# highlando/optconpy

Measured on AMD Instinct MI355X. Metric: ADI shift-solves/sec (wall-clock to feedback K in ms_per_step), higher is better.
Workload: dtype f64

## Files before the change

### include/ricadi.h

```cpp
#ifndef RICADI_H
#define RICADI_H

#include <stdint.h>

#ifdef __cplusplus
extern "C" {
#endif

#define RICADI_OK 0
#define RICADI_EINVAL (-1)
#define RICADI_EHIP (-2)
#define RICADI_ENOCONV (-3)
#define RICADI_EBREAKDOWN (-4)
#define RICADI_ESTATE (-5)

typedef struct ricadi_ctx ricadi_ctx;

#define RICADI_MAX_HIERARCHY_LEVELS 6

typedef struct ricadi_opts {
  double gmres_tol;
  int gmres_restart;
  int gmres_maxit;
  int bj_block;
// ... 39 lines not shown
                        const int32_t* a_rowptr, const int32_t* a_col, const double* a_val,
                        const int32_t* e_rowptr, const int32_t* e_col, const double* e_val,
                        const int32_t* j_rowptr, const int32_t* j_col, const double* j_val);

int ricadi_clear_cache(ricadi_ctx* ctx);

int ricadi_set_dims(ricadi_ctx* ctx, int nv);

int ricadi_set_lowrank(ricadi_ctx* ctx, const double* U, const double* V, int q);

int ricadi_spmm(ricadi_ctx* ctx, double alpha, double beta,
                const double* X, int m, double* Y);

int ricadi_precond_apply(ricadi_ctx* ctx, double alpha, double beta,
                         const double* R, int m, double* Z);

#define RICADI_PCF_H16 (1 << 0)
#define RICADI_PCF_X32 (1 << 1)
#define RICADI_PCF_MID32 (1 << 2)
#define RICADI_PCF_B16 (1 << 3)
#define RICADI_PCF_RESTRICT_SHIFT 4
#define RICADI_PCF_COARSE_SHIFT 6
#define RICADI_PCF_PFUSED (1 << 8)
#define RICADI_PCF_PSPLIT (1 << 9)
#define RICADI_PCF_FIRST_SHIFT 10
#define RICADI_PCF_LAST_SHIFT 12
#define RICADI_PCF_FOLDED (1 << 14)
#define RICADI_PCF_VANKA (1 << 15)
#define RICADI_PCF_TWO_KS_SHIFT 16
#define RICADI_PCF_RECT_KS_SHIFT 24
int ricadi_precond_apply_batch_dev(ricadi_ctx* ctx, int ng, const double* alphas, const double* betas,
                                   const double* dR, int64_t r_stride, int m, const int32_t* active,
                                   int nactive, double* dZ, int* form_out);

#define RICADI_OA_X32 1
#define RICADI_OA_Y32 2
#define RICADI_OA_LOWRANK 4
#define RICADI_OA_RESIDUAL 8
int ricadi_op_apply_batch_dev(ricadi_ctx* ctx, int ng, const double* alphas, const double* betas, const double* dX,
                              int64_t x_stride, int m, const int32_t* active, int nactive, int flags, double alpha,
                              const double* dR, int64_t r_stride, double beta_r, double* dY, int64_t y_stride,
                              int* variant_out);

int ricadi_precond_structure(ricadi_ctx* ctx, int level, int32_t* sizes_out, int32_t* bv_ptr, int32_t* bv_rows,
                             int32_t* bp_ptr, int32_t* bp_rows, int32_t* aggof, int32_t* p_rp, int32_t* p_ci,
                             double* p_v);

int ricadi_precond_vanka(ricadi_ctx* ctx, int level, int32_t* sizes_out, int32_t* colour_ptr, int32_t* patch_idx);

int ricadi_shift_solve(ricadi_ctx* ctx, double alpha, double beta,
                       const double* R, const double* Rp, int m,
                       double* X_out, int* iters_out, double* relres_out);

int ricadi_lyap_adi(ricadi_ctx* ctx, const double* shifts, int nshifts,
                    const double* W, int m, const ricadi_adi_params* prm,
                    double* Z_out, int* c_out, double* stats_out);

int ricadi_ric_newtonadi(ricadi_ctx* ctx, const double* shifts, int nshifts,
                         const double* B, int nb, const double* W, int mw,
                         const double* Z0, int c0, const double* oldB,
                         const ricadi_adi_params* prm,
                         double* Z_out, int zcap, int* c_out, double* stats_out);

int ricadi_compress(ricadi_ctx* ctx, const double* Z, int c, double thresh, int kmax,
                    double* Zc_out, int* k_out, double* sv_out);

// ... 59 lines not shown
#define RICADI_TK_ITER_SPLIT 18
#define RICADI_TK_PC_VANKA 19
int ricadi_time_kernel_dev(ricadi_ctx* ctx, int which, int ng, const double* alphas,
                           const double* betas, int m, int nvec, int reps,
                           double* ms_per_launch);

int ricadi_qr(ricadi_ctx* ctx, const double* Z, int c, double* Q_out, double* R_out);

int ricadi_project_pencil(ricadi_ctx* ctx, const double* Q, int k, double* HA, double* HE);
int ricadi_project_pencil_dev(ricadi_ctx* ctx, const double* dQ, int k, double* dHA, double* dHE);

int ricadi_setup_info(ricadi_ctx* ctx, int* out, int nout);

int ricadi_dense_inverse_batch(ricadi_ctx* ctx, int k, int nb, double* A, int* route_out);

int ricadi_time_qr_dev(ricadi_ctx* ctx, const double* dZ, int c, int reps, double* ms_per_call);

int ricadi_time_gram_dev(ricadi_ctx* ctx, const double* dZ, int c, double* dG, int reps,
                         double* ms_per_launch);

int ricadi_set_recycle(ricadi_ctx* ctx, int depth);

typedef int (*ricadi_allgather_fn)(void* user, const void* send_dev, void* recv_dev,
                                   int64_t bytes_per_rank);
int ricadi_set_exchange(ricadi_ctx* ctx, int rank, int world, ricadi_allgather_fn fn, void* user,
                        void* send_dev, void* recv_dev, int64_t send_capacity);

int ricadi_rccl_unique_id(void* id_out, int bytes);
int ricadi_set_exchange_rccl(ricadi_ctx* ctx, int rank, int world, const void* unique_id, void* comm,
                             int64_t send_capacity);
int ricadi_exchange_count(ricadi_ctx* ctx, int64_t* count_out);

int ricadi_host_deal(const double* shifts, int nshifts, int world, int32_t* owner_out);
int ricadi_host_sa_criterion(int nv, const int32_t* a_rowptr, const int32_t* a_col, const double* a_val,
                             double* rowsum_ratio_out, double* skew_ratio_out, int* on_out);
int ricadi_host_plan_levels(int nv, int np, const int32_t* a_rowptr, const int32_t* a_col, const double* a_val,
                            const int32_t* e_rowptr, const int32_t* e_col, const double* e_val,
                            const int32_t* j_rowptr, const int32_t* j_col, const double* j_val,
                            const ricadi_opts* opts, int32_t* out);
int ricadi_host_plan_hierarchy(int nv, int np, const int32_t* a_rowptr, const int32_t* a_col, const double* a_val,
                               const int32_t* e_rowptr, const int32_t* e_col, const double* e_val,
                               const int32_t* j_rowptr, const int32_t* j_col, const double* j_val,
                               const ricadi_opts* opts, int32_t* nlevels_out, int32_t* levels_out,
                               int32_t* smoothed_out);
int ricadi_host_saddle_tiles(int nv, int np, const int32_t* a_rowptr, const int32_t* a_col, const double* a_val,
                             const int32_t* e_rowptr, const int32_t* e_col, const double* e_val,
                             const int32_t* j_rowptr, const int32_t* j_col, const double* j_val,
                             const ricadi_opts* opts, int32_t* sizes_out, int32_t* rows2, int32_t* rp2,
                             int32_t* cols2, uint16_t* lidx, uint16_t* lidx_ms, double* vAJ, double* vE,
                             int32_t* perm, int32_t* s_rp, int32_t* s_ci, double* s_src);
int ricadi_host_vanka_patches(int nv, int np, const int32_t* j_rowptr, const int32_t* j_col, const double* j_val,
                              int32_t* sizes_out, int32_t* colour_ptr, int32_t* patch_idx);
int ricadi_host_aggregate(int n, const int32_t* rowptr, const int32_t* col,
                          int bsize, int32_t* blk_out);
int ricadi_host_cauchy(const double* shifts, int g, double* rinv_out, double* cinv1_out);

#ifdef __cplusplus
}
#endif
#endif
```

### optconpy_amd/_lib.py

```python
from __future__ import annotations

import ctypes as C
import os

import numpy as np
import scipy.sparse as sps

_HERE = os.path.dirname(os.path.abspath(__file__))
LIB_PATH = os.environ.get("RICADI_LIB", os.path.join(_HERE, "libricadi_hip.so"))

RICADI_OK = 0
RICADI_ENOCONV = -3
MAX_M = 128
ABI_VERSION = 403


class RicadiOpts(C.Structure):
    _fields_ = [("gmres_tol", C.c_double), ("gmres_restart", C.c_int),
                ("gmres_maxit", C.c_int), ("bj_block", C.c_int), ("agg_v", C.c_int),
                ("agg_p", C.c_int), ("coarse_max", C.c_int), ("use_coarse", C.c_int),
                ("max_levels", C.c_int), ("verbose", C.c_int), ("compress_qr", C.c_int),
                ("hierarchy", C.c_int), ("child_smoother", C.c_int), ("child_damping", C.c_double)]


class RicadiAdiParams(C.Structure):
    _fields_ = [("adi_max_steps", C.c_int), ("adi_newZ_reltol", C.c_double),
                ("nwtn_max_steps", C.c_int), ("nwtn_upd_reltol", C.c_double),
                ("nwtn_upd_abstol", C.c_double), ("project_w", C.c_int),
                ("verbose", C.c_int), ("compress_cols", C.c_int), ("sweep_width", C.c_int)]


_dp = C.POINTER(C.c_double)
_ip = C.POINTER(C.c_int32)
_vp = C.c_void_p
_up = C.POINTER(C.c_uint16)

SIGNATURES = {
    "ricadi_last_error": (C.c_char_p, []),
    "ricadi_version": (C.c_int, []),
    "ricadi_sizeof_opts": (C.c_int, []),
    "ricadi_sizeof_adi_params": (C.c_int, []),
    "ricadi_struct_signature": (C.c_char_p, []),
    "ricadi_default_opts": (None, [C.POINTER(RicadiOpts)]),
    "ricadi_default_adi_params": (None, [C.POINTER(RicadiAdiParams)]),
    "ricadi_create": (C.c_int, [C.c_int, C.POINTER(_vp)]),
    "ricadi_destroy": (C.c_int, [_vp]),
    "ricadi_set_opts": (C.c_int, [_vp, C.POINTER(RicadiOpts)]),
# ... 27 lines not shown
    "ricadi_spmm_dev": (C.c_int, [_vp, C.c_double, C.c_double, _vp, C.c_int, _vp]),
    "ricadi_shift_solve_dev": (C.c_int, [_vp, C.c_double, C.c_double, _vp, C.c_int, _vp,
                                         C.POINTER(C.c_int), _dp]),
    "ricadi_shift_solve_batch_dev": (C.c_int, [_vp, C.c_int, _dp, _dp, _vp, C.c_int64, C.c_int, _vp,
                                               C.POINTER(C.c_int), _dp]),
    "ricadi_time_spmm_batch_dev": (C.c_int, [_vp, C.c_int, _dp, _dp, _vp, C.c_int, _vp, C.c_int,
                                             C.POINTER(C.c_double)]),
    "ricadi_sweep_recombine_dev": (C.c_int, [_vp, C.c_int, _vp, C.c_int, _dp, _dp, _vp, _vp,
                                             C.POINTER(C.c_double)]),
    "ricadi_sweep_recombine_slots_dev": (C.c_int, [_vp, C.c_int, C.c_int, _vp, C.c_int, _dp, _dp, _vp, _vp,
                                                   C.POINTER(C.c_double), _dp]),
    "ricadi_apply_e_dev": (C.c_int, [_vp, C.c_double, _vp, C.c_int, _vp]),
    "ricadi_lincomb_dev": (C.c_int, [_vp, C.c_int, C.c_int, C.c_int, _vp, C.c_int64, _dp, _vp]),
    "ricadi_gain_dev": (C.c_int, [_vp, C.c_double, _vp, C.c_int, C.c_int, _vp, C.c_int, _vp]),
    "ricadi_panel_norms_dev": (C.c_int, [_vp, _vp, C.c_int, C.c_int, _dp, _dp]),
    "ricadi_time_spmm_dev": (C.c_int, [_vp, C.c_double, C.c_double, _vp, C.c_int, _vp, C.c_int,
                                       _dp]),
    "ricadi_time_kernel_dev": (C.c_int, [_vp, C.c_int, C.c_int, _dp, _dp, C.c_int, C.c_int, C.c_int,
                                         C.POINTER(C.c_double)]),
    "ricadi_qr": (C.c_int, [_vp, _dp, C.c_int, _dp, _dp]),
    "ricadi_project_pencil": (C.c_int, [_vp, _dp, C.c_int, _dp, _dp]),
    "ricadi_project_pencil_dev": (C.c_int, [_vp, _vp, C.c_int, _vp, _vp]),
    "ricadi_setup_info": (C.c_int, [_vp, C.POINTER(C.c_int), C.c_int]),
    "ricadi_time_qr_dev": (C.c_int, [_vp, _vp, C.c_int, C.c_int, C.POINTER(C.c_double)]),
    "ricadi_time_gram_dev": (C.c_int, [_vp, _vp, C.c_int, _vp, C.c_int, _dp]),
    "ricadi_set_recycle": (C.c_int, [_vp, C.c_int]),
    "ricadi_set_exchange": (C.c_int, [_vp, C.c_int, C.c_int, _vp, _vp, _vp, _vp, C.c_int64]),
    "ricadi_rccl_unique_id": (C.c_int, [_vp, C.c_int]),
    "ricadi_set_exchange_rccl": (C.c_int, [_vp, C.c_int, C.c_int, _vp, _vp, C.c_int64]),
    "ricadi_exchange_count": (C.c_int, [_vp, C.POINTER(C.c_int64)]),
    "ricadi_dense_inverse_batch": (C.c_int, [_vp, C.c_int, C.c_int, _dp, C.POINTER(C.c_int)]),
    "ricadi_precond_apply_batch_dev": (C.c_int, [_vp, C.c_int, _dp, _dp, _vp, C.c_int64, C.c_int, _ip, C.c_int,
                                                 _vp, C.POINTER(C.c_int)]),
    "ricadi_precond_structure": (C.c_int, [_vp, C.c_int, _ip, _ip, _ip, _ip, _ip, _ip, _ip, _ip, _dp]),
    "ricadi_op_apply_batch_dev": (C.c_int, [_vp, C.c_int, _dp, _dp, _vp, C.c_int64, C.c_int, _ip, C.c_int, C.c_int,
                                            C.c_double, _vp, C.c_int64, C.c_double, _vp, C.c_int64,
                                            C.POINTER(C.c_int)]),
    "ricadi_host_saddle_tiles": (C.c_int, [C.c_int, C.c_int, _ip, _ip, _dp, _ip, _ip, _dp, _ip, _ip, _dp,
                                           C.POINTER(RicadiOpts), _ip, _ip, _ip, _ip, _up, _up, _dp, _dp, _ip, _ip,
                                           _ip, _dp]),
    "ricadi_host_deal": (C.c_int, [_dp, C.c_int, C.c_int, _ip]),
    "ricadi_host_sa_criterion": (C.c_int, [C.c_int, _ip, _ip, _dp, C.POINTER(C.c_double), C.POINTER(C.c_double),
                                           C.POINTER(C.c_int)]),
    "ricadi_host_plan_levels": (C.c_int, [C.c_int, C.c_int, _ip, _ip, _dp, _ip, _ip, _dp, _ip, _ip, _dp,
                                          C.POINTER(RicadiOpts), _ip]),
    "ricadi_host_plan_hierarchy": (C.c_int, [C.c_int, C.c_int, _ip, _ip, _dp, _ip, _ip, _dp, _ip, _ip, _dp,
                                             C.POINTER(RicadiOpts), _ip, _ip, _ip]),
    "ricadi_host_aggregate": (C.c_int, [C.c_int, _ip, _ip, C.c_int, _ip]),
    "ricadi_host_vanka_patches": (C.c_int, [C.c_int, C.c_int, _ip, _ip, _dp, _ip, _ip, _ip]),
    "ricadi_precond_vanka": (C.c_int, [_vp, C.c_int, _ip, _ip, _ip]),
    "ricadi_host_cauchy": (C.c_int, [_dp, C.c_int, _dp, _dp]),
}

EXCHANGE_FN = C.CFUNCTYPE(C.c_int, _vp, _vp, _vp, C.c_int64)

_lib = None


def load():
    global _lib
    if _lib is not None:
        return _lib
    if not os.path.exists(LIB_PATH):
        raise RuntimeError(
            "libricadi_hip.so is missing ({0}); build it with "
            "`python -c 'import __graft_entry__ as g; g.build()'` -- there is no "
# ... 465 lines not shown

    def shift_solve_batch_dev(self, alphas, betas, r_ptr, r_stride, m, x_ptr, strict=True):
        al = np.ascontiguousarray(alphas, dtype=np.float64)
        be = np.ascontiguousarray(betas, dtype=np.float64)
        ng = al.size
        its = (C.c_int * ng)()
        rr = np.zeros((ng, m))
        rc = self._lib.ricadi_shift_solve_batch_dev(self._h, ng, _d(al), _d(be), r_ptr,
                                                    int(r_stride), m, x_ptr, its, _d(rr))
        _chk(rc, allow_noconv=not strict)
        return list(its), rr

    def time_spmm_batch_dev(self, alphas, betas, x_ptr, m, y_ptr, reps):
        al = np.ascontiguousarray(alphas, dtype=np.float64)
        be = np.ascontiguousarray(betas, dtype=np.float64)
        ms = C.c_double(0.0)
        _chk(self._lib.ricadi_time_spmm_batch_dev(self._h, al.size, _d(al), _d(be), x_ptr, m, y_ptr,
                                                  reps, C.byref(ms)))
        return ms.value

    TK = dict(spmm=0, block_v=1, block_p=2, coarse=3, spmm_sy=4, dots=5, update_dots=6, update=7,
              precond=8, restrict=9, pc_restrict=10, pc_coarse=11, pc_sy_prows=12, pc_two_term=13,
              pc_jprod=14, pc_schur=15, pc_rect=16, iter=17, iter_split=18, pc_vanka=19)

    def time_kernel_dev(self, which, alphas, betas, m, nvec=7, reps=100):
        al = np.ascontiguousarray(alphas, dtype=np.float64)
        be = np.ascontiguousarray(betas, dtype=np.float64)
        ms = C.c_double(0.0)
        _chk(self._lib.ricadi_time_kernel_dev(self._h, int(self.TK.get(which, which)), al.size, _d(al),
                                              _d(be), int(m), int(nvec), int(reps), C.byref(ms)))
        return ms.value

    def setup_info(self):
        a = (C.c_int * 30)()
        _chk(self._lib.ricadi_setup_info(self._h, a, 30))
        return dict(zip(("nv", "np", "nbv", "nbp", "bs", "kc", "spmm_row_blocks", "spmm_max_cols", "levels",
                         "dense_coarse", "fp16_vector_input", "rect_ks", "two_term_ks", "np_", "nnz_j",
                         "nnz_sy", "nnz_restriction", "coarse_route", "k1_variant", "fp32_intermediate", "fp32_operator_output",
                         "child_smoother", "vanka_colours", "vanka_patches", "vanka_largest_patch", "vanka_dropped",
                         "vanka_lone_patches", "hierarchy", "hierarchy_levels", "hierarchy_dense"),
                        list(a)))

    def dense_inverse_batch(self, mats):
        A = np.ascontiguousarray(mats, dtype=np.float64).copy()
        if A.ndim != 3 or A.shape[1] != A.shape[2]:
            raise ValueError("mats must be nb x k x k")
        route = C.c_int(-1)
        _chk(self._lib.ricadi_dense_inverse_batch(self._h, A.shape[1], A.shape[0], _d(A), C.byref(route)))
        return A, int(route.value)

    PCF_RESTRICT = {0: None, 1: "rowwave", 2: "csr16", 3: "csr64"}
    PCF_COARSE = {0: None, 1: "child", 2: "dense"}
    PCF_FIRST = {0: None, 1: "two32", 2: "two_term", 3: "plain"}
    PCF_LAST = {0: None, 1: "rect32", 2: "rect", 3: "csr_in"}

    @classmethod
    def decode_precond_form(cls, w):
        w &= 0xFFFFFFFF
        return dict(h16=bool(w & 1), x32=bool(w & 2), mid32=bool(w & 4), b16=bool(w & 8),
                    restrict=cls.PCF_RESTRICT[(w >> 4) & 3], coarse=cls.PCF_COARSE[(w >> 6) & 3],
                    pfused=bool(w & (1 << 8)), psplit=bool(w & (1 << 9)), first=cls.PCF_FIRST[(w >> 10) & 3],
                    last=cls.PCF_LAST[(w >> 12) & 3], folded=bool(w & (1 << 14)), vanka=bool(w & (1 << 15)),
                    two_term_ks=(w >> 16) & 255,
                    rect_ks=(w >> 24) & 255)

    def precond_apply_batch_dev(self, alphas, betas, r_ptr, r_stride, m, z_ptr, active=None):
        al = np.ascontiguousarray(alphas, dtype=np.float64)
        be = np.ascontiguousarray(betas, dtype=np.float64)
        act = None if active is None else np.ascontiguousarray(active, dtype=np.int32)
        form = C.c_int(-1)
        _chk(self._lib.ricadi_precond_apply_batch_dev(self._h, al.size, _d(al), _d(be), r_ptr, int(r_stride), int(m),
                                                      None if act is None else _i(act),
                                                      0 if act is None else act.size, z_ptr, C.byref(form)))
        return self.decode_precond_form(form.value)

    OA_X32, OA_Y32, OA_LOWRANK, OA_RESIDUAL = 1, 2, 4, 8

    def op_apply_batch_dev(self, alphas, betas, x_ptr, x_stride, m, y_ptr, y_stride, active=None, flags=0,
                           alpha=1.0, r_ptr=None, r_stride=0, beta_r=0.0):
        al = np.ascontiguousarray(alphas, dtype=np.float64)
        be = np.ascontiguousarray(betas, dtype=np.float64)
        act = None if active is None else np.ascontiguousarray(active, dtype=np.int32)
        var = C.c_int(-1)
        _chk(self._lib.ricadi_op_apply_batch_dev(self._h, al.size, _d(al), _d(be), x_ptr, int(x_stride), int(m),
                                                 None if act is None else _i(act), 0 if act is None else act.size,
                                                 int(flags), float(alpha), r_ptr, int(r_stride), float(beta_r),
                                                 y_ptr, int(y_stride), C.byref(var)))
        return int(var.value)

    def precond_structure(self, level=0):
        sz = np.zeros(16, dtype=np.int32)
        nul = [None] * 8
        _chk(self._lib.ricadi_precond_structure(self._h, int(level), _i(sz), *nul))
        nv, np_, nbv, nbp, bs, kc, kcv, kcp, sa, nnzp, child, folded, rect, p32, agg_v, agg_p = (int(x) for x in sz)
        n = nv + np_
        out = dict(bv_ptr=np.zeros(nbv + 1, np.int32), bv_rows=np.zeros(nv, np.int32),
                   bp_ptr=np.zeros(nbp + 1, np.int32), bp_rows=np.zeros(np_, np.int32),
                   aggof=np.zeros(n if kc > 0 else 0, np.int32), p_rp=np.zeros(n + 1, np.int32),
                   p_ci=np.zeros(nnzp, np.int32), p_v=np.zeros(nnzp))
        ptr = lambda a: _d(a) if a.dtype == np.float64 else _i(a)
        _chk(self._lib.ricadi_precond_structure(self._h, int(level), _i(sz), *[ptr(out[k]) for k in (
            "bv_ptr", "bv_rows", "bp_ptr", "bp_rows", "aggof", "p_rp", "p_ci", "p_v")]))
        P = (sps.csr_matrix((out.pop("p_v"), out.pop("p_ci"), out.pop("p_rp")), shape=(n, kc)) if kc > 0 else None)
        if nbp == 0:
            out["bp_ptr"] = np.zeros(1, np.int32)
        out.update(nv=nv, np=np_, nbv=nbv, nbp=nbp, bs=bs, kc=kc, kcv=kcv, kcp=kcp, smoothed=bool(sa), P=P,
                   child=bool(child), folded=bool(folded), rect=bool(rect), precond32=bool(p32), agg_v=agg_v,
# ... 88 lines not shown

def _vanka_records(call):
    sz = np.zeros(8, dtype=np.int32)
    _chk(call(_i(sz), None, None))
    ncol, npat = int(sz[0]), int(sz[1])
    cp = np.zeros(ncol + 1, dtype=np.int32)
    idx = np.full((npat, 64), -1, dtype=np.int32)
    _chk(call(_i(sz), _i(cp), _i(idx)))
    return dict(colours=ncol, patches=npat, pressure_patches=int(sz[2]), largest=int(sz[3]), dropped=int(sz[4]),
                lone=int(sz[5]), lone_patches=int(sz[6]), colour_ptr=cp, patch_idx=idx)


def host_vanka_patches(nv, J):
    J = sps.csr_matrix(J, dtype=np.float64)
    if J.shape[1] != nv:
        raise ValueError("J has the wrong number of columns")
    rp = np.ascontiguousarray(J.indptr, dtype=np.int32)
    ci = np.ascontiguousarray(J.indices, dtype=np.int32)
    v = np.ascontiguousarray(J.data, dtype=np.float64)
    lib = load()
    return _vanka_records(lambda sz, cp, pi: lib.ricadi_host_vanka_patches(int(nv), J.shape[0], _i(rp), _i(ci),
                                                                           _d(v), sz, cp, pi))


def host_aggregate(pattern, bsize):
    rp, ci, _, sh = as_csr(pattern)
    blk = np.empty(sh[0], dtype=np.int32)
    nb = load().ricadi_host_aggregate(sh[0], _i(rp), _i(ci), int(bsize), _i(blk))
    if nb < 0:
        _chk(nb)
    return blk, nb


def host_deal(shifts, world):
    sh = np.ascontiguousarray(shifts, dtype=np.float64)
    owner = np.empty(sh.size, dtype=np.int32)
    _chk(load().ricadi_host_deal(_d(sh), sh.size, int(world), _i(owner)))
    return owner


def host_cauchy(shifts):
    sh = np.ascontiguousarray(shifts, dtype=np.float64)
    g = sh.size
    rinv = np.empty((g, g))
    c1 = np.empty(g)
    _chk(load().ricadi_host_cauchy(_d(sh), g, _d(rinv), _d(c1)))
    return rinv, c1


def host_plan_levels(calA, calE, J, **opts):
    a, e, j = as_csr(calA), as_csr(calE), as_csr(J)
    o = default_opts(**opts)
    out = np.zeros(5, dtype=np.int32)
    _chk(load().ricadi_host_plan_levels(a[3][0], j[3][0], _i(a[0]), _i(a[1]), _d(a[2]), _i(e[0]), _i(e[1]), _d(e[2]),
                                        _i(j[0]), _i(j[1]), _d(j[2]), C.byref(o), _i(out)))
    return dict(levels=int(out[0]), kc=int(out[1]), kcv=int(out[2]), kcp=int(out[3]), smoothed=bool(out[4]))


PLAN_KEYS = ("nv", "np", "kv", "kp", "agg_v", "agg_p", "has_child", "dense_dim")
MAX_HIERARCHY_LEVELS = 6


def host_plan_hierarchy(calA, calE, J, **opts):
    a, e, j = as_csr(calA), as_csr(calE), as_csr(J)
    o = default_opts(**opts)
    nlev = np.zeros(1, dtype=np.int32)
# ... 45 lines not shown
```

### optconpy_amd/csrc/ricadi_ctx.h

```cpp
#pragma once
#include <rccl/rccl.h>
#include <rocsolver/rocsolver.h>

#include <chrono>
#include <cmath>
#include <future>
#include <numeric>
#include <cstdio>
#include <cstdlib>
#include <cstring>
#include <memory>
#include <tuple>

#include "ricadi_internal.h"

namespace ricadi {

extern thread_local std::string g_err;

struct HipError {
  std::string msg;
};
#define HIPCHK(expr)                                                                      \
  do {                                                                                    \
// ... 169 lines not shown
  DArr<double> v;
  void upload(const HostCsr& h, hipStream_t st) {
    nrows = h.nrows;
    rp.upload(h.rp, st);
    ci.upload(h.ci, st);
    v.upload(h.v, st);
  }
};

struct Exec {
  hipStream_t st = nullptr;
  rocblas_handle rb = nullptr;
  DevPool* pool = nullptr;
  int* info = nullptr;
  int* flag = nullptr;
};

struct Switches {
  bool precond64 = false;
  bool basis64 = false;
  bool basis32 = false;
  bool timing = false;
  bool debug_sweeps = false;
  bool smw = true;
  bool wide_split = true;
  double sa_omega = 0.5;
  bool sweep_meta = true;
  bool ms_spmm = true;
  bool ms_force = false;
  bool w32 = true;
  bool x32_always = true;
  bool blocks16 = true;
  bool rowwave = true;
  bool mid32 = true;
  bool coarse_pipe = true;
  bool lowsync = true;
  bool split = true;
  bool setup_overlap = true;
};

}

using namespace ricadi;

struct ricadi_ctx {
  int dev = 0;
  hipStream_t st = nullptr;
  rocblas_handle rb = nullptr;
  std::unique_ptr<ricadi_ctx> child;
  bool borrowed = false;
  int levels = 2;
  ricadi_opts opts;
  Switches sw;
  bool has_op = false;
  int nv = 0, np = 0, n = 0;
  int bs = 32, nbv = 0, nbp = 0, kc = 0;
  int agg_v = 0, agg_p = 0;
  size_t snnz = 0;
  DArr<int> s_rp, s_ci;
  DArr<double> srcA, srcE, srcJ;
  DevCsr A, E, J, JT;
  DArr<int> bv_ptr, bv_rows, bp_ptr, bp_rows, jd_ptr, jd_vblk;
  DArr<int> ps_meta;
  DArr<int> sw_meta;
  int sw_stride = 0, sw_in_rect = 0, sw_in_two = 0;
  DArr<double> bvA, bvE, jd_val;
// ... 1 lines not shown
  bool ady_ok = false;
  int ady_ks = 0;
  DArr<int> cy_ptr, cy_cols;
  DArr<double> cy_dA, cy_dE, cy_dJ, cy_dT;
  bool sa = false;
  DArr<int> pt_rp, pt_ci;
  DArr<double> pt_v;
  bool vanka = false;
  VankaPatches vk;
  DArr<int> vk_idx;
  bool gt_ok = false;
  int gt_ks = 0;
  DArr<int> gt_ptr, gt_cols;
  DArr<double> gt_jtd;
  DArr<double> E0, EM, EJ, ones;
  size_t synnz = 0;
  int sy_chunk = 16;
  DArr<int> sy_rp, sy_ci;
  DArr<double> sy_A, sy_E, sy_J;
  int syb_max_cols = 0;
  bool syb_ok = false;
  DArr<int> syb_rp2, syb_cols2, syb_perm;
  DArr<uint16_t> syb_lidx;
  int sb_nblk = 0, sb_max_cols = 0, sb_max_nnz = 0;
  bool sb_ok = false;
  DArr<int> sb_perm;
  DArr<int> sb_rows2, sb_rp2, sb_cols2, sb_colsm2;
  DArr<uint16_t> sb_lidx;
  DArr<double> sbAJ, sbE, sybAJ, sybE;
  DArr<uint16_t> sb_lidx_ms, syb_lidx_ms;
  bool ms_ok = false;
  int w32_last = -1;
  int mid32_last = -1;
  int q = 0;
  DArr<double> U, V, lrc, scratch;
  long lr_epoch = 0;
  DArr<double> smw_rhs, smw_x, smw_cap;
  DArr<double> split_b, split_x;
  DArr<double> sweep_u, sweep_t, sweep_coef, sweep_part;
  std::map<std::pair<double, double>, std::unique_ptr<ShiftData>> cache;
  int wcols = 0, wrestart = 0;
  DArr<double> basis, vcur, wv, zv, r2, tp, rc, ec, xs, bvec, pw1, pw2;
  DArr<float> basisf, zbasisf;
  DArr<float> wv32;
  bool basis32 = true;
  bool basis16 = true;
  bool precond32 = true;
  DArr<double> partial, h1, h2, H, cs, sn, g, scale, resid, yv, bnorm2, nrm2;
  DArr<double> ls_partial, ls_coef;
  DArr<int> flag, ipiv, info;
  DArr<double*> eptrs;
  DArr<double> gj_cb, gj_rp, gj_rb, gj_d;
  DArr<double*> gj_ptrs;
  double** gj_hptrs = nullptr;
  size_t gj_hcap = 0;
  DArr<int> flag2;
  double* h_resid = nullptr;
  hipEvent_t ev_res[2] = {nullptr, nullptr};
  hipStream_t st_half = nullptr;
  hipEvent_t ev_res_half[2] = {nullptr, nullptr};
  hipEvent_t ev_fork = nullptr, ev_join = nullptr;
  DArr<double> Z;
  int zc = 0, zld = 0;
  DevPool pool;
  hipStream_t st2 = nullptr;
  rocblas_handle rb2 = nullptr;
// ... 56 lines not shown
```

### optconpy_amd/csrc/ricadi_host.cpp

```cpp
#include <array>
#include <cmath>
#include <cstdio>
#include <cstdlib>
#include <cstring>
#include <numeric>
#include <stdexcept>

#include "ricadi_internal.h"

namespace ricadi {

HostCsr make_csr(int nrows, int ncols, const int32_t* rp, const int32_t* ci, const double* v) {
  HostCsr a;
  a.nrows = nrows;
  a.ncols = ncols;
  a.rp.assign(rp, rp + nrows + 1);
  const int nnz = rp[nrows];
  a.ci.assign(ci, ci + nnz);
  a.v.assign(v, v + nnz);
  sort_rows(a);
  return a;
}

void sort_rows(HostCsr& a) {
// ... 1159 lines not shown
    };
    out(rows2, r.sb_rows2, (size_t)nb * 32);
    out(rp2, r.sb_rp2, (size_t)nb * 33);
    out(cols2, r.sb_cols2, (size_t)nb * mc);
    out(lidx, hs.sb_lidx, nnz);
    out(perm, hs.sb_perm, nnz);
    out(s_rp, hs.s_rp, (size_t)hs.n + 1);
    out(s_ci, hs.s_ci, nnz);
    if (s_src) {
      out(s_src, hs.s_srcA, nnz);
      out(s_src + nnz, hs.s_srcE, nnz);
      out(s_src + 2 * nnz, hs.s_srcJ, nnz);
    }
    if (r.ms_ok) {
      out(lidx_ms, r.sb_lidx_ms, nnz);
      out(vAJ, r.sbAJ, nnz);
      out(vE, r.sbE, nnz);
    }
  } catch (...) {
    ricadi::set_error("ricadi_host_saddle_tiles: exception");
    return RICADI_EINVAL;
  }
  return RICADI_OK;
}

int ricadi_host_deal(const double* shifts, int ns, int world, int32_t* owner_out) {
  if (!shifts || !owner_out || ns < 1 || world < 1) {
    ricadi::set_error("ricadi_host_deal: bad argument");
    return RICADI_EINVAL;
  }
  return ricadi::deal_shifts(shifts, ns, world, owner_out);
}

int ricadi_host_cauchy(const double* shifts, int g, double* rinv_out, double* cinv1_out) {
  if (!shifts || !rinv_out || !cinv1_out) {
    ricadi::set_error("ricadi_host_cauchy: bad argument");
    return RICADI_EINVAL;
  }
  int rc = ricadi::cauchy_data(shifts, g, rinv_out, cinv1_out);
  if (rc == RICADI_EBREAKDOWN)
    ricadi::set_error("ricadi_host_cauchy: Cauchy matrix not positive definite "
                      "(shifts must be distinct, negative and few)");
  return rc;
}

}
```

### optconpy_amd/csrc/ricadi_internal.h

```cpp
#pragma once
#include <hip/hip_runtime.h>

#include <algorithm>
#include <cstddef>
#include <cstdint>
#include <map>
#include <string>
#include <utility>
#include <vector>

#include "../../include/ricadi.h"

#define RICADI_MAX_M 128
#define RICADI_MAX_GROUPS 16

namespace ricadi {

struct HostCsr {
  int nrows = 0, ncols = 0;
  std::vector<int> rp, ci;
  std::vector<double> v;
  size_t nnz() const { return ci.size(); }
};
HostCsr make_csr(int nrows, int ncols, const int32_t* rp, const int32_t* ci, const double* v);
// ... 133 lines not shown
  const int* meta = nullptr;
  int stride = 0, in_off = 0;
};

struct LowRankArgs {
  const double* U = nullptr;
  const double* c = nullptr;
  size_t gsc = 0;
  int q = 0, nrows = 0;
};

struct CsrInArgs {
  const int* rp = nullptr;
  const int* ci = nullptr;
  GroupPtrs v = {};
  const double* src = nullptr;
  size_t gss = 0;
  const double* base = nullptr;
  size_t gsb = 0;
  double scale = 1.0;
};

struct Seg2 {
  const int* iptr = nullptr;
  const int* irows = nullptr;
  const int* moff = nullptr;
  int kstride = 0;
  const double* in = nullptr;
  size_t gs = 0;
  const _Float16* in16 = nullptr;
};

bool spmm_rowwave_pays(int nrows, size_t nnz);
void launch_spmm_rowwave(hipStream_t st, const GroupTab& gt, int nrows, const int* rp, const int* ci,
                         const GroupPtrs& vals, const double* x, const _Float16* x16, size_t gsx, double* y, size_t gsy,
                         int m, bool kb = false);
__host__ __device__ inline size_t rckb_index(int j, int c, int k) {
  return j < (k & ~3) ? ((size_t)(j >> 2) * 16 + c) * 4 + (j & 3) : (size_t)j * 16 + c;
}

void launch_spmm_h(hipStream_t st, const GroupTab& gt, int nrows, const int* rp, const int* ci,
                   const GroupPtrs& vals, const double* x, const _Float16* x16, int ldx, size_t gsx, double* y, int ldy,
                   size_t gsy, const _Float16* r16, int ldr, size_t gsr, double alpha, double beta_r, int m, int chunk);
void launch_spmm_b(hipStream_t st, const GroupTab& gt, int nrows, const int* rp, const int* ci,
                   const GroupPtrs& vals, const double* x, int ldx, size_t gsx, const int* xmap,
                   double* y, int ldy, size_t gsy, const double* r, int ldr, size_t gsr,
                   double alpha, double beta_r, int m, const LowRankArgs& lr = LowRankArgs(),
                   int chunk = 16);
void launch_spmm_blocked_b(hipStream_t st, const GroupTab& gt, int nblk, const int* rows2,
                           const int* rp2, const int* cols2, const uint16_t* lidx,
                           const GroupPtrs& vals, const double* x, int ldx, size_t gsx, double* y,
                           int ldy, size_t gsy, const double* r, int ldr, size_t gsr, double alpha,
                           double beta_r, int m, int max_cols,
                           const LowRankArgs& lr = LowRankArgs());
bool spmm_blocked_ms_ok(int m, int max_cols, size_t panel_rows);
void launch_spmm_blocked_x32(hipStream_t st, const GroupTab& gt, int nblk, const int* rows2, const int* rp2,
                             const int* cols2, const uint16_t* lidx, const GroupPtrs& vals, const float* x, int ldx,
                             size_t gsx, double* y, int ldy, size_t gsy, double alpha, int m, int max_cols, float* y32 = nullptr);
void launch_spmm_blocked_ms_x32(hipStream_t st, const GroupTab& gt, const double* alphas, const double* betas,
                                int nblk, const int* rows2, const int* rp2, const int* cols2, const uint16_t* lidx,
                                const double* vAJ, const double* vE, const float* x, int ldx, size_t gsx, double* y,
                                int ldy, size_t gsy, double alpha, int m, int max_cols, float* y32 = nullptr);
void launch_spmm_blocked_ms(hipStream_t st, const GroupTab& gt, const double* alphas, const double* betas,
                            int nblk, const int* rows2, const int* rp2, const int* cols2,
                            const uint16_t* lidx, const double* vAJ, const double* vE,
                            const double* x, int ldx, size_t gsx, double* y, int ldy, size_t gsy,
                            const double* r, int ldr, size_t gsr, double alpha, double beta_r, int m,
                            int max_cols);
void launch_axpby_b(hipStream_t st, const GroupTab& gt, size_t n, double a, const double* x,
// ... 193 lines not shown
```

### optconpy_amd/csrc/ricadi_spmm.hip

```cpp
#include "ricadi_device.h"

namespace ricadi {

__device__ __forceinline__ double lowrank_term(const LowRankArgs& lr, const double* __restrict__ lrc,
                                               int row, int col, int m) {
  const double* __restrict__ u = lr.U + (size_t)row * lr.q;
  double s = 0.0;
  for (int k = 0; k < lr.q; ++k) s = fma(u[k], lrc[k * m + col], s);
  return s;
}

template <int CPL, int CHK, class XT = double, class RT = double>
__global__ __launch_bounds__(256) void spmm_kernel_v2(
    GroupTab gt, int nrows, const int* __restrict__ rp, const int* __restrict__ ci,
    GroupPtrs vals, const XT* __restrict__ x, int ldx, size_t gsx,
    const int* __restrict__ xmap, double* __restrict__ y, int ldy, size_t gsy,
    const RT* __restrict__ r, int ldr, size_t gsr, double alpha, double beta_r,
    const double* __restrict__ rowscale, int m, LowRankArgs lr) {
  const int grp = gt.gid[blockIdx.z];
  const double* __restrict__ val = vals.p[grp];
  x += (size_t)grp * gsx;
  y += (size_t)grp * gsy;
  if (r) r += (size_t)grp * gsr;
  const double* __restrict__ lrc = lr.c + (size_t)grp * lr.gsc;
  const int nwg = gridDim.x, orig = blockIdx.x;
  const int qd = nwg >> 3, rm = nwg & 7, xcd = orig & 7;
  const int blk = (xcd < rm ? xcd * (qd + 1) : rm * (qd + 1) + (xcd - rm) * qd) + (orig >> 3);
  const int g = threadIdx.x & 15;
  const int row = blk * 16 + (threadIdx.x >> 4);
  const bool live = row < nrows;
  double acc[CPL];
  int colx[CPL];
// ... 183 lines not shown
        acc[1] = fma(myv[u], a.y, acc[1]);
        acc[2] = fma(myv[u], b.x, acc[2]);
        acc[3] = fma(myv[u], b.y, acc[3]);
        acc[4] = fma(myv[u], c2.x, acc[4]);
        acc[5] = fma(myv[u], c2.y, acc[5]);
        acc[6] = fma(myv[u], d.x, acc[6]);
        acc[7] = fma(myv[u], d.y, acc[7]);
      }
    }
  }
#pragma unroll
  for (int t = 0; t < 8; ++t) {
    double v = acc[t];
    v += rw_dpp<0xB1>(v);
    v += rw_dpp<0x4E>(v);
    v += rw_dpp<0x141>(v);
    v += rw_dpp<0x140>(v);
    v += __shfl_xor(v, 16, 64);
    acc[t] = v;
  }
  if (KB && row < (nrows & ~3)) {
    double v = acc[0];
#pragma unroll
    for (int t = 1; t < 8; ++t) v = e == t ? acc[t] : v;
    if (e < 8) y[rckb_index(row, h * 8 + e, nrows)] = v;
  } else if (e == 0) {
    double2* o = reinterpret_cast<double2*>(y + (size_t)row * 16 + h * 8);
    o[0] = make_double2(acc[0], acc[1]);
    o[1] = make_double2(acc[2], acc[3]);
    o[2] = make_double2(acc[4], acc[5]);
    o[3] = make_double2(acc[6], acc[7]);
  }
}
bool spmm_rowwave_pays(int nrows, size_t nnz) { return nrows > 0 && nnz >= (size_t)32 * nrows; }
void launch_spmm_rowwave(hipStream_t st, const GroupTab& gt, int nrows, const int* rp, const int* ci,
                         const GroupPtrs& vals, const double* x, const _Float16* x16, size_t gsx, double* y, size_t gsy,
                         int m, bool kb) {
  if (nrows <= 0 || m != 16 || gt.ng <= 0) return;
  dim3 grid((nrows + 3) / 4, 1, gt.ng), block(256);
#define RW_LAUNCH(XT, KB, X) \
  hipLaunchKernelGGL((spmm_rowwave_kernel<XT, KB>), grid, block, 0, st, gt, nrows, rp, ci, vals, X, gsx, y, gsy)
  if (x16 && kb) RW_LAUNCH(_Float16, true, x16);
  else if (x16) RW_LAUNCH(_Float16, false, x16);
  else if (kb) RW_LAUNCH(double, true, x);
  else RW_LAUNCH(double, false, x);
#undef RW_LAUNCH
}

template <bool HAS_R, bool HAS_LR, class XT = double, bool F4 = false>
__global__ __launch_bounds__(256) void spmm_blocked_kernel(
    const int* __restrict__ rows2, const int* __restrict__ rp2, const int* __restrict__ cols2,
    const uint16_t* __restrict__ lidx, GroupTab gt, GroupPtrs vals,
    const XT* __restrict__ x, int ldx, size_t gsx,
    double* __restrict__ y, int ldy, size_t gsy, const double* __restrict__ r, int ldr,
    size_t gsr, double alpha, double beta_r, int m, int max_cols, LowRankArgs lr, float* __restrict__ y32) {
  extern __shared__ double xs[];
  const int grp = gt.gid[blockIdx.z];
  const double* __restrict__ val = vals.p[grp];
  x += (size_t)grp * gsx;
  y += (size_t)grp * gsy;
  if (y32) y32 += (size_t)grp * gsy;
  if (HAS_R) r += (size_t)grp * gsr;
  const double* __restrict__ lrc = HAS_LR ? lr.c + (size_t)grp * lr.gsc : nullptr;
  const int nwg = gridDim.x, orig = blockIdx.x;
  const int qd = nwg >> 3, rm = nwg & 7, xcd = orig & 7;
  const int b = (xcd < rm ? xcd * (qd + 1) : rm * (qd + 1) + (xcd - rm) * qd) + (orig >> 3);
  const int g = threadIdx.x & 15, gq = threadIdx.x >> 4;
  const int* __restrict__ bcols = cols2 + (size_t)b * max_cols;
  constexpr int NR = 2, NCH = 3;
  int ka[NR], kb[NR], grow[NR];
  double myv[NR][NCH];
  int myl[NR][NCH];
#pragma unroll
  for (int rr = 0; rr < NR; ++rr) {
    const int q = gq + 16 * rr;
    ka[rr] = rp2[b * 33 + q];
    kb[rr] = rp2[b * 33 + q + 1];
    grow[rr] = rows2[b * 32 + q];
  }
// ... 523 lines not shown
```

Before: 871.3.

## Add multi-row-per-wave rowwave SpMM kernel with prefetch and quad k-blocked stores

Adds a spmm_rowrun kernel in which each wavefront walks several consecutive CSR rows, prefetching the next batch of column/value entries across row boundaries, and in the k-blocked layout writes four rows at once as double2 stores. A heuristic picks rows-per-wave so the grid still holds enough waves, and new debug/test entry points expose restriction and the rowwave kernel. The aim is to amortise per-wave launch overhead and row-length latency on the restriction SpMM, at the risk of lower parallelism and more register use. A ctx flag rowrun defaults to false, and the launcher's callers shown here do not pass rows, so whether the new path runs by default is unclear.

Measured after the change: 861.2. -1.2%, worse.

```diff
diff --git a/include/ricadi.h b/include/ricadi.h
--- a/include/ricadi.h
+++ b/include/ricadi.h
@@ -95,6 +95,15 @@
 int ricadi_precond_apply_batch_dev(ricadi_ctx* ctx, int ng, const double* alphas, const double* betas,
                                    const double* dR, int64_t r_stride, int m, const int32_t* active,
                                    int nactive, double* dZ, int* form_out);
+
+int ricadi_precond_restrict_dev(ricadi_ctx* ctx, int ng, const double* alphas, const double* betas, const double* dR,
+                                int64_t r_stride, int m, const int32_t* active, int nactive, double* dRc,
+                                int* form_out, int* kblocked_out, int* rows_out);
+
+int ricadi_spmm_rowwave_dev(ricadi_ctx* ctx, int nrows, const int32_t* d_rowptr, const int32_t* d_col,
+                            const double* d_val, const void* dX, int x_fp16, int64_t x_stride, int ng,
+                            const int32_t* active, int nactive, double* dY, int64_t y_stride, int kblocked, int rows,
+                            int* rows_out);
 
 #define RICADI_OA_X32 1
 #define RICADI_OA_Y32 2
@@ -220,6 +229,7 @@
 int ricadi_exchange_count(ricadi_ctx* ctx, int64_t* count_out);
 
 int ricadi_host_deal(const double* shifts, int nshifts, int world, int32_t* owner_out);
+int ricadi_host_restrict_rows(int nrows, int ng, int* rows_out);
 int ricadi_host_sa_criterion(int nv, const int32_t* a_rowptr, const int32_t* a_col, const double* a_val,
                              double* rowsum_ratio_out, double* skew_ratio_out, int* on_out);
 int ricadi_host_plan_levels(int nv, int np, const int32_t* a_rowptr, const int32_t* a_col, const double* a_val,
diff --git a/optconpy_amd/_lib.py b/optconpy_amd/_lib.py
--- a/optconpy_amd/_lib.py
+++ b/optconpy_amd/_lib.py
@@ -12,7 +12,7 @@
 RICADI_OK = 0
 RICADI_ENOCONV = -3
 MAX_M = 128
-ABI_VERSION = 403
+ABI_VERSION = 404
 
 
 class RicadiOpts(C.Structure):
@@ -106,6 +106,11 @@
     "ricadi_dense_inverse_batch": (C.c_int, [_vp, C.c_int, C.c_int, _dp, C.POINTER(C.c_int)]),
     "ricadi_precond_apply_batch_dev": (C.c_int, [_vp, C.c_int, _dp, _dp, _vp, C.c_int64, C.c_int, _ip, C.c_int,
                                                  _vp, C.POINTER(C.c_int)]),
+    "ricadi_precond_restrict_dev": (C.c_int, [_vp, C.c_int, _dp, _dp, _vp, C.c_int64, C.c_int, _ip, C.c_int, _vp,
+                                              C.POINTER(C.c_int), C.POINTER(C.c_int), C.POINTER(C.c_int)]),
+    "ricadi_spmm_rowwave_dev": (C.c_int, [_vp, C.c_int, _vp, _vp, _vp, _vp, C.c_int, C.c_int64, C.c_int, _ip, C.c_int,
+                                          _vp, C.c_int64, C.c_int, C.c_int, C.POINTER(C.c_int)]),
+    "ricadi_host_restrict_rows": (C.c_int, [C.c_int, C.c_int, C.POINTER(C.c_int)]),
     "ricadi_precond_structure": (C.c_int, [_vp, C.c_int, _ip, _ip, _ip, _ip, _ip, _ip, _ip, _ip, _dp]),
     "ricadi_op_apply_batch_dev": (C.c_int, [_vp, C.c_int, _dp, _dp, _vp, C.c_int64, C.c_int, _ip, C.c_int, C.c_int,
                                             C.c_double, _vp, C.c_int64, C.c_double, _vp, C.c_int64,
@@ -637,13 +642,14 @@
         return ms.value
 
     def setup_info(self):
-        a = (C.c_int * 30)()
-        _chk(self._lib.ricadi_setup_info(self._h, a, 30))
+        a = (C.c_int * 31)()
+        _chk(self._lib.ricadi_setup_info(self._h, a, 31))
         return dict(zip(("nv", "np", "nbv", "nbp", "bs", "kc", "spmm_row_blocks", "spmm_max_cols", "levels",
                          "dense_coarse", "fp16_vector_input", "rect_ks", "two_term_ks", "np_", "nnz_j",
                          "nnz_sy", "nnz_restriction", "coarse_route", "k1_variant", "fp32_intermediate", "fp32_operator_output",
                          "child_smoother", "vanka_colours", "vanka_patches", "vanka_largest_patch", "vanka_dropped",
-                         "vanka_lone_patches", "hierarchy", "hierarchy_levels", "hierarchy_dense"),
+                         "vanka_lone_patches", "hierarchy", "hierarchy_levels", "hierarchy_dense",
+                         "restrict_rows"),
                         list(a)))
 
     def dense_inverse_batch(self, mats):
@@ -678,6 +684,26 @@
                                                       None if act is None else _i(act),
                                                       0 if act is None else act.size, z_ptr, C.byref(form)))
         return self.decode_precond_form(form.value)
+
+    def precond_restrict_dev(self, alphas, betas, r_ptr, r_stride, m, rc_ptr, active=None):
+        al = np.ascontiguousarray(alphas, dtype=np.float64)
+        be = np.ascontiguousarray(betas, dtype=np.float64)
+        act = None if active is None else np.ascontiguousarray(active, dtype=np.int32)
+        form, kb, rows = C.c_int(-1), C.c_int(-1), C.c_int(-1)
+        _chk(self._lib.ricadi_precond_restrict_dev(self._h, al.size, _d(al), _d(be), r_ptr, int(r_stride), int(m),
+                                                   None if act is None else _i(act), 0 if act is None else act.size,
+                                                   rc_ptr, C.byref(form), C.byref(kb), C.byref(rows)))
+        return self.decode_precond_form(form.value), bool(kb.value), rows.value
+
+    def spmm_rowwave_dev(self, nrows, rp_ptr, ci_ptr, val_ptr, x_ptr, x_fp16, x_stride, ng, y_ptr, y_stride,
+                         kblocked=False, rows=0, active=None):
+        act = None if active is None else np.ascontiguousarray(active, dtype=np.int32)
+        ran = C.c_int(-1)
+        _chk(self._lib.ricadi_spmm_rowwave_dev(self._h, int(nrows), rp_ptr, ci_ptr, val_ptr, x_ptr, int(bool(x_fp16)),
+                                               int(x_stride), int(ng), None if act is None else _i(act),
+                                               0 if act is None else act.size, y_ptr, int(y_stride),
+                                               int(bool(kblocked)), int(rows), C.byref(ran)))
+        return ran.value
 
     OA_X32, OA_Y32, OA_LOWRANK, OA_RESIDUAL = 1, 2, 4, 8
 
@@ -832,6 +858,22 @@
     return blk, nb
 
 
+def rckb_rows(panel):
+    flat = np.asarray(panel).reshape(-1)
+    k = flat.size // 16
+    k4 = k & ~3
+    out = np.empty((k, 16), dtype=flat.dtype)
+    out[:k4] = flat[:k4 * 16].reshape(k4 // 4, 16, 4).transpose(0, 2, 1).reshape(k4, 16)
+    out[k4:] = flat[k4 * 16:].reshape(k - k4, 16)
+    return out
+
+
+def host_restrict_rows(nrows, ng):
+    r = C.c_int(0)
+    _chk(load().ricadi_host_restrict_rows(int(nrows), int(ng), C.byref(r)))
+    return r.value
+
+
 def host_deal(shifts, world):
     sh = np.ascontiguousarray(shifts, dtype=np.float64)
     owner = np.empty(sh.size, dtype=np.int32)
diff --git a/optconpy_amd/csrc/ricadi_ctx.h b/optconpy_amd/csrc/ricadi_ctx.h
--- a/optconpy_amd/csrc/ricadi_ctx.h
+++ b/optconpy_amd/csrc/ricadi_ctx.h
@@ -225,6 +225,7 @@
   bool x32_always = true;
   bool blocks16 = true;
   bool rowwave = true;
+  bool rowrun = false;
   bool mid32 = true;
   bool coarse_pipe = true;
   bool lowsync = true;
@@ -292,6 +293,7 @@
   bool ms_ok = false;
   int w32_last = -1;
   int mid32_last = -1;
+  int restrict_rows_last = -1;
   int q = 0;
   DArr<double> U, V, lrc, scratch;
   long lr_epoch = 0;
diff --git a/optconpy_amd/csrc/ricadi_host.cpp b/optconpy_amd/csrc/ricadi_host.cpp
--- a/optconpy_amd/csrc/ricadi_host.cpp
+++ b/optconpy_amd/csrc/ricadi_host.cpp
@@ -1215,6 +1215,15 @@
   return ricadi::deal_shifts(shifts, ns, world, owner_out);
 }
 
+int ricadi_host_restrict_rows(int nrows, int ng, int* rows_out) {
+  if (!rows_out || nrows < 1 || ng < 1) {
+    ricadi::set_error("ricadi_host_restrict_rows: bad argument");
+    return RICADI_EINVAL;
+  }
+  *rows_out = ricadi::spmm_rowwave_rows(nrows, ng);
+  return RICADI_OK;
+}
+
 int ricadi_host_cauchy(const double* shifts, int g, double* rinv_out, double* cinv1_out) {
   if (!shifts || !rinv_out || !cinv1_out) {
     ricadi::set_error("ricadi_host_cauchy: bad argument");
diff --git a/optconpy_amd/csrc/ricadi_internal.h b/optconpy_amd/csrc/ricadi_internal.h
--- a/optconpy_amd/csrc/ricadi_internal.h
+++ b/optconpy_amd/csrc/ricadi_internal.h
@@ -189,9 +189,15 @@
 };
 
 bool spmm_rowwave_pays(int nrows, size_t nnz);
-void launch_spmm_rowwave(hipStream_t st, const GroupTab& gt, int nrows, const int* rp, const int* ci,
-                         const GroupPtrs& vals, const double* x, const _Float16* x16, size_t gsx, double* y, size_t gsy,
-                         int m, bool kb = false);
+int launch_spmm_rowwave(hipStream_t st, const GroupTab& gt, int nrows, const int* rp, const int* ci,
+                        const GroupPtrs& vals, const double* x, const _Float16* x16, size_t gsx, double* y, size_t gsy,
+                        int m, bool kb = false, int rows = 0);
+inline int spmm_rowwave_rows(int nrows, int ng) {
+  if (nrows < 1) return 1;
+  for (int rows = 8; rows > 1; rows >>= 1)
+    if ((long long)((nrows - 1) / rows + 1) * ng >= 2048) return rows;
+  return 1;
+}
 __host__ __device__ inline size_t rckb_index(int j, int c, int k) {
   return j < (k & ~3) ? ((size_t)(j >> 2) * 16 + c) * 4 + (j & 3) : (size_t)j * 16 + c;
 }
diff --git a/optconpy_amd/csrc/ricadi_spmm.hip b/optconpy_amd/csrc/ricadi_spmm.hip
--- a/optconpy_amd/csrc/ricadi_spmm.hip
+++ b/optconpy_amd/csrc/ricadi_spmm.hip
@@ -1,3 +1,5 @@
+#include <stdexcept>
+
 #include "ricadi_device.h"
 
 namespace ricadi {
@@ -247,19 +249,166 @@
     o[3] = make_double2(acc[6], acc[7]);
   }
 }
+template <class XT, bool KB, bool QUAD>
+__global__ __launch_bounds__(256) void spmm_rowrun_kernel(
+    GroupTab gt, int nrows, int rows, const int* __restrict__ rp, const int* __restrict__ ci, GroupPtrs vals,
+    const XT* __restrict__ x, size_t gsx, double* __restrict__ y, size_t gsy) {
+  static_assert(KB || !QUAD, "the four-row store is the k-blocked layout's");
+  const int grp = gt.gid[blockIdx.z];
+  const double* __restrict__ val = vals.p[grp];
+  x += (size_t)grp * gsx;
+  y += (size_t)grp * gsy;
+  const int row0 = (blockIdx.x * 4 + (threadIdx.x >> 6)) * rows;
+  if (row0 >= nrows) return;
+  const int nr = min(rows, nrows - row0);
+  const int lane = threadIdx.x & 63, e = lane & 31, h = lane >> 5;
+  const int pv = rp[row0 + min(lane, nr)];
+  double acc[8];
+#pragma unroll
+  for (int t = 0; t < 8; ++t) acc[t] = 0.0;
+  constexpr int NB = 4;
+  int cn[NB];
+  double vn[NB];
+  auto fetch = [&](int kb, int k1) {
+#pragma unroll
+    for (int u = 0; u < NB; ++u) {
+      const int k = kb + 32 * u + e;
+      cn[u] = ci[min(k, k1 - 1)];
+      const double v = val[min(k, k1 - 1)];
+      vn[u] = k < k1 ? v : 0.0;
+    }
+  };
+  double q4[4] = {0.0, 0.0, 0.0, 0.0};
+  auto flush = [&](int row) {
+#pragma unroll
+    for (int t = 0; t < 8; ++t) {
+      double v = acc[t];
+      v += rw_dpp<0xB1>(v);
+      v += rw_dpp<0x4E>(v);
+      v += rw_dpp<0x141>(v);
+      v += rw_dpp<0x140>(v);
+      v += __shfl_xor(v, 16, 64);
+      acc[t] = v;
+    }
+    if (KB && row < (nrows & ~3)) {
+      double v = acc[0];
+#pragma unroll
+      for (int t = 1; t < 8; ++t) v = e == t ? acc[t] : v;
+      if constexpr (QUAD) {
+        const int j = row & 3;
+#pragma unroll
+        for (int t = 0; t < 4; ++t) q4[t] = j == t ? v : q4[t];
+        if (j == 3 && e < 8) {
+          double2* o = reinterpret_cast<double2*>(y + rckb_index(row - 3, h * 8 + e, nrows));
+          o[0] = make_double2(q4[0], q4[1]);
+          o[1] = make_double2(q4[2], q4[3]);
+        }
+      } else {
+        if (e < 8) y[rckb_index(row, h * 8 + e, nrows)] = v;
+      }
+    } else if (e == 0) {
+      double2* o = reinterpret_cast<double2*>(y + (size_t)row * 16 + h * 8);
+      o[0] = make_double2(acc[0], acc[1]);
+      o[1] = make_double2(acc[2], acc[3]);
+      o[2] = make_double2(acc[4], acc[5]);
+      o[3] = make_double2(acc[6], acc[7]);
+    }
+#pragma unroll
+    for (int t = 0; t < 8; ++t) acc[t] = 0.0;
+  };
+  bool have = false;
+  for (int r = 0; r < nr; ++r) {
+    const int k0 = __builtin_amdgcn_readlane(pv, r), k1 = __builtin_amdgcn_readlane(pv, r + 1);
+    const int nbatch = (k1 - k0 + 32 * NB - 1) / (32 * NB);
+    if (nbatch > 0 && !have) fetch(k0, k1);
+    have = false;
+    if (nbatch == 0 && r > 0) flush(row0 + r - 1);
+    for (int bi = 0; bi < nbatch; ++bi) {
+      int myc[NB];
+      double myv[NB];
+#pragma unroll
+      for (int u = 0; u < NB; ++u) {
+        myc[u] = cn[u];
+        myv[u] = vn[u];
+      }
+      auto fetch_next = [&]() {
+        if (bi + 1 < nbatch) {
+          fetch(k0 + (bi + 1) * 32 * NB, k1);
+        } else if (r + 1 < nr) {
+          const int k2 = __builtin_amdgcn_readlane(pv, r + 2);
+          if (k2 > k1) {
+            fetch(k1, k2);
+            have = true;
+          }
+        }
+      };
+      if constexpr (sizeof(XT) == 2) {
+        rw_half8 xv[NB];
+#pragma unroll
+        for (int u = 0; u < NB; ++u) xv[u] = *reinterpret_cast<const rw_half8*>(x + (size_t)myc[u] * 16 + h * 8);
+        fetch_next();
+        if (bi == 0 && r > 0) flush(row0 + r - 1);
+#pragma unroll
+        for (int u = 0; u < NB; ++u)
+#pragma unroll
+          for (int t = 0; t < 8; ++t) acc[t] = fma(myv[u], (double)xv[u][t], acc[t]);
+      } else {
+        fetch_next();
+        if (bi == 0 && r > 0) flush(row0 + r - 1);
+#pragma unroll
+        for (int u = 0; u < NB; ++u) {
+          const double2* xp = reinterpret_cast<const double2*>(x + (size_t)myc[u] * 16 + h * 8);
+          const double2 a = xp[0], b = xp[1], c2 = xp[2], d = xp[3];
+          acc[0] = fma(myv[u], a.x, acc[0]);
+          acc[1] = fma(myv[u], a.y, acc[1]);
+          acc[2] = fma(myv[u], b.x, acc[2]);
+          acc[3] = fma(myv[u], b.y, acc[3]);
+          acc[4] = fma(myv[u], c2.x, acc[4]);
+          acc[5] = fma(myv[u], c2.y, acc[5]);
+          acc[6] = fma(myv[u], d.x, acc[6]);
+          acc[7] = fma(myv[u], d.y, acc[7]);
+        }
+      }
+    }
+  }
+  flush(row0 + nr - 1);
+}
 bool spmm_rowwave_pays(int nrows, size_t nnz) { return nrows > 0 && nnz >= (size_t)32 * nrows; }
-void launch_spmm_rowwave(hipStream_t st, const GroupTab& gt, int nrows, const int* rp, const int* ci,
-                         const GroupPtrs& vals, const double* x, const _Float16* x16, size_t gsx, double* y, size_t gsy,
-                         int m, bool kb) {
-  if (nrows <= 0 || m != 16 || gt.ng <= 0) return;
-  dim3 grid((nrows + 3) / 4, 1, gt.ng), block(256);
+int launch_spmm_rowwave(hipStream_t st, const GroupTab& gt, int nrows, const int* rp, const int* ci,
+                        const GroupPtrs& vals, const double* x, const _Float16* x16, size_t gsx, double* y, size_t gsy,
+                        int m, bool kb, int rows) {
+  if (nrows <= 0 || m != 16 || gt.ng <= 0) return 0;
+  if (rows == 0) rows = spmm_rowwave_rows(nrows, gt.ng);
+  if (rows != 1 && rows != 2 && rows != 4 && rows != 8) throw std::invalid_argument("spmm_rowwave: rows per wave");
+  dim3 grid((nrows - 1) / (4 * rows) + 1, 1, gt.ng), block(256);
+  if (rows == 1) {
 #define RW_LAUNCH(XT, KB, X) \
   hipLaunchKernelGGL((spmm_rowwave_kernel<XT, KB>), grid, block, 0, st, gt, nrows, rp, ci, vals, X, gsx, y, gsy)
-  if (x16 && kb) RW_LAUNCH(_Float16, true, x16);
-  else if (x16) RW_LAUNCH(_Float16, false, x16);
-  else if (kb) RW_LAUNCH(double, true, x);
-  else RW_LAUNCH(double, false, x);
+    if (x16 && kb) RW_LAUNCH(_Float16, true, x16);
+    else if (x16) RW_LAUNCH(_Float16, false, x16);
+    else if (kb) RW_LAUNCH(double, true, x);
+    else RW_LAUNCH(double, false, x);
 #undef RW_LAUNCH
+    return rows;
+  }
+  const bool quad = kb && rows >= 4;
+  if (quad) {
+    for (int j = 0; j < 4; ++j)
+      if (rckb_index(4 + j, 5, 8) != rckb_index(4, 5, 8) + j || rckb_index(4, 5, 8) % 2)
+        throw std::logic_error("spmm_rowwave: the k-blocked layout is not four rows of a column side by side");
+    if (reinterpret_cast<uintptr_t>(y) % 16 || gsy % 2) throw std::invalid_argument("spmm_rowwave: y not 16-byte aligned");
+  }
+#define RW_LAUNCH(XT, KB, QUAD, X)                                                                                \
+  hipLaunchKernelGGL((spmm_rowrun_kernel<XT, KB, QUAD>), grid, block, 0, st, gt, nrows, rows, rp, ci, vals, X, gsx, \
+                     y, gsy)
+  if (x16 && quad) RW_LAUNCH(_Float16, true, true, x16);
+  else if (x16 && kb) RW_LAUNCH(_Float16, true, false, x16);
+  else if (x16) RW_LAUNCH(_Float16, false, false, x16);
+  else if (quad) RW_LAUNCH(double, true, true, x);
+  else if (kb) RW_LAUNCH(double, true, false, x);
+  else RW_LAUNCH(double, false, false, x);
+#undef RW_LAUNCH
+  return rows;
 }
 
 template <bool HAS_R, bool HAS_LR, class XT = double, bool F4 = false>
```
